# DigitalPhonetics/Intrinsic-Subgraph-Generation-for-VQA

Measured on AMD Instinct MI355X. Metric: GQA questions/sec, higher is better.
Workload: dtype f32

## Files before the change

intrinsic-subgraph-generation-for-vqa_amd/csrc/isg_layer_conv.hip:

```cpp
#include "isg_f16x3.hpp"

#include "isg_diag.hpp"
#include "isg_live_tables.hpp"
#include "../../include/isg_masked.h"

ISG_DIAG_BUFFER(g_lc_stamps)
#define LC_STAMP(i) ISG_DIAG_ADD(i)

namespace isg {

typedef __attribute__((address_space(3))) void lc_lds_t;
typedef __attribute__((address_space(1))) void lc_glb_t;

constexpr int LC_ROWS = 64, LC_ECAP = 256, LC_C = 128, LC_K = 128, LC_LDX = LC_C + 4, LC_LDA = LC_K + 8, LC_THREADS = 512;
constexpr int LC_OFF_XR = LC_ROWS * LC_LDX * 4;
constexpr int LC_OFF_A = 2 * LC_ROWS * LC_LDX * 4;
constexpr int LC_OFF_TAB = LC_OFF_A + 2 * 64 * LC_LDA * 2;
constexpr int LC_OFF_RAW = LC_OFF_TAB + 2 * (LC_ECAP * 16 + LC_ECAP * 4 + 68 * 4) + LC_ECAP * 4 + 4 * 64 * 4 + 64 * 4 + 3 * LC_C * 4 +
                           4 * LC_C * 4;
constexpr int LC_OFF_LIVE = LC_OFF_RAW + LC_ROWS * LC_K * 4;
constexpr int LC_SMEM_BYTES = LC_OFF_LIVE + 2 * 4 * 8;
static_assert(LC_OFF_RAW % 16 == 0, "16-byte pieces");
static_assert(LC_SMEM_BYTES <= 160 * 1024, "one workgroup per CU");

// ... 155 lines not shown
      const isg_f32x2 va = gelu_exact2(isg_f32x2{(acc[i][4 * g] * si) * wi4[g][0] + bv4[g][0], (acc[i][4 * g + 1] * si) * wi4[g][1] + bv4[g][1]});
      const isg_f32x2 vb = gelu_exact2(isg_f32x2{(acc[i][4 * g + 2] * si) * wi4[g][2] + bv4[g][2], (acc[i][4 * g + 3] * si) * wi4[g][3] + bv4[g][3]});
      *reinterpret_cast<hf32x4 *>(&sC[row][wave * 32 + 8 * g + 4 * hh]) = hf32x4{va.x, va.y, vb.x, vb.y};
    }
  }
  __syncthreads();
  const int grp = lane >> 4, l = lane & 15;
#pragma unroll
  for (int it = 0; it < 4; ++it) {
    const int n = wave * 16 + it * 4 + grp;
    float part = 0.f;
    if (n < nrows) {
      const float *qr = q + (int64_t)s_b[n] * NG_C;
      part += dot4_rn(*reinterpret_cast<const float4 *>(&sC[n][4 * l]), *reinterpret_cast<const float4 *>(qr + 4 * l));
      part += dot4_rn(*reinterpret_cast<const float4 *>(&sC[n][4 * (l + 16)]), *reinterpret_cast<const float4 *>(qr + 4 * (l + 16)));
    }
    const float dot = group_sum<16>(part);
    if (n < nrows && l == 0) gate[r0 + n] = gelu_libm(dot / denom);
  }
}

#define LC_EPILOGUE_ARITH(SL01, XS, XD)                                                                              \
    float part[4];                                                                                                   \
    int cb = tw * 32 + 4 * hh;        \
    asm volatile("" : "+v"(cb));                                                                                     \
    _Pragma("unroll") for (int g = 0; g < 4; ++g) {                                                                  \
      const int cc = cb + 8 * g;                                                                                     \
      const float4 xl4 = *reinterpret_cast<const float4 *>(&sXl[XS][cc]);                                            \
      const float4 xr4 = *reinterpret_cast<const float4 *>(&sXr[XD][cc]);                                            \
      const float4 at4 = *reinterpret_cast<const float4 *>(&s_att[cc]);                                              \
      const float4 wi4 = *reinterpret_cast<const float4 *>(&s_weinv[cc]);                                            \
      const float lv[4] = {xl4.x, xl4.y, xl4.z, xl4.w}, rv[4] = {xr4.x, xr4.y, xr4.z, xr4.w};                        \
      const float atv[4] = {at4.x, at4.y, at4.z, at4.w}, wiv[4] = {wi4.x, wi4.y, wi4.z, wi4.w};                      \
      part[g] = 0.f;                                                                                                 \
      _Pragma("unroll") for (int jj = 0; jj < 4; ++jj) {                                                             \
        const float e = (acc[g * 4 + jj] * sinv) * wiv[jj];                                                          \
        float z = (rv[jj] + lv[jj]) + e;                                                                             \
        if (MASKED) z *= me;                                                                                         \
        z = (SL01) ? fmaxf(z, z * slope) : (z > 0.f ? z : z * slope);    \
        if (MASKED) z *= me;                                                                                         \
        part[g] = fmaf(z, atv[jj], part[g]);                                                                         \
      }                                                                                                              \
      if (g < 3) __builtin_amdgcn_sched_barrier(0);                                                                  \
    }                                                                                                                \
    const float mine = (part[0] + part[1]) + (part[2] + part[3]);                                                    \
    const float tot = mine + __shfl_xor(mine, 32);                                                                   \
    if (hh == 0) s_part[tw * 64 + prow] = tot;

#define LC_AGGREGATE(REC)                                                                                                                  \
  {                                                                                                                                        \
    const int q8 = lane >> 3, j8 = lane & 7;                                                                                               \
    const int k = 8 * wave + q8;                                                                                                           \
    if (k < nrows) {                                                                                                                       \
      const int rb = s_rp[k], re = min(s_rp[k + 1], ne);                                                                                   \
      float lg4[4], e4[4];                                                                                                                 \
      int4 rc4[4];                                                                                                                         \
    _Pragma("unroll")                                                                                                                      \
      for (int u = 0; u < 4; ++u) {                                                                                                        \
        const int idx = max(min(rb + u, re - 1), 0);                                                                                       \
        lg4[u] = s_lg[idx];                                                                                                                \
        rc4[u] = REC(idx);                                                                                                                 \
      }                                                                                                                                    \
      float4 u2[2][4];                                                \
    _Pragma("unroll")                                                                                                                      \
      for (int u = 0; u < 2; ++u)                                                                                                          \
    _Pragma("unroll")                                                                                                                      \
        for (int m = 0; m < 4; ++m) u2[u][m] = *reinterpret_cast<const float4 *>(&sXl[rc4[u].x][32 * m + j8 * 4]);                         \
      float mx = fmaxf(fmaxf(-INFINITY, lg4[0]), fmaxf(fmaxf(lg4[1], lg4[2]), lg4[3]));                                                    \
    _Pragma("unroll 1")                                                                                                                    \
      for (int s = rb + 4; s < re; s += 4) {                                                                                               \
        const float v0 = s_lg[s], v1 = s_lg[min(s + 1, re - 1)], v2 = s_lg[min(s + 2, re - 1)], v3 = s_lg[min(s + 3, re - 1)];             \
        mx = fmaxf(fmaxf(mx, v0), fmaxf(fmaxf(v1, v2), v3));                                                                               \
      }                                                                                                                                    \
      float den = 0.f;                                             \
    _Pragma("unroll")                                                                                                                      \
      for (int u = 0; u < 4; ++u) {                                                                                                        \
        e4[u] = __builtin_amdgcn_exp2f((lg4[u] - mx) * 1.4426950408889634f);                                                               \
        den += rb + u < re ? e4[u] : 0.f;                                                                                                  \
      }                                                                                                                                    \
    _Pragma("unroll 1")                                                                                                                    \
      for (int s = rb + 4; s < re; s += 4) {                                                                                               \
        const float v0 = s_lg[s], v1 = s_lg[min(s + 1, re - 1)], v2 = s_lg[min(s + 2, re - 1)], v3 = s_lg[min(s + 3, re - 1)];             \
        const float e0 = __builtin_amdgcn_exp2f((v0 - mx) * 1.4426950408889634f);                                                          \
        const float e1 = __builtin_amdgcn_exp2f((v1 - mx) * 1.4426950408889634f);                                                          \
        const float e2 = __builtin_amdgcn_exp2f((v2 - mx) * 1.4426950408889634f);                                                          \
        const float e3 = __builtin_amdgcn_exp2f((v3 - mx) * 1.4426950408889634f);                                                          \
        den += e0;                                                                                                                         \
        den += s + 1 < re ? e1 : 0.f;                                                                                                      \
        den += s + 2 < re ? e2 : 0.f;                                                                                                      \
        den += s + 3 < re ? e3 : 0.f;                                                                                                      \
      }                                                                                                                                    \
      const float rden = __builtin_amdgcn_rcpf(den + 1e-16f);                                                                              \
      float4 o[4];                                                                                                                         \
    _Pragma("unroll")                                                                                                                      \
      for (int m = 0; m < 4; ++m) o[m] = make_float4(0.f, 0.f, 0.f, 0.f);                                                                  \
      int s = rb;                                                                                                                          \
    _Pragma("unroll 1")                                                                                                                    \
      while (true) {           \
        {                                           \
          const float wsel = (j8 & 2) ? ((j8 & 1) ? e4[3] : e4[2]) : ((j8 & 1) ? e4[1] : e4[0]);                                           \
          const int esel = (j8 & 2) ? ((j8 & 1) ? rc4[3].y : rc4[2].y) : ((j8 & 1) ? rc4[1].y : rc4[0].y);                                 \
          if (j8 < 4 && s + j8 < re) a.alpha[(int64_t)esel * a.H + hd] = wsel * rden;                                                      \
        }                                                                                                                                  \
    _Pragma("unroll")                                                                                                                      \
        for (int hp = 0; hp < 2; ++hp) {                                                                                                   \
          if (hp == 1) {                    \
// ... 11 lines not shown
            const float wm = MASKED ? mul_rn(w, __int_as_float(rc4[2 * hp + u].w)) : w;                                                    \
    _Pragma("unroll")                                                                                                                      \
            for (int m = 0; m < 4; ++m) {                                                                                                  \
              o[m].x = fmaf(u2[u][m].x, wm, o[m].x);                                                                                       \
              o[m].y = fmaf(u2[u][m].y, wm, o[m].y);                                                                                       \
              o[m].z = fmaf(u2[u][m].z, wm, o[m].z);                                                                                       \
              o[m].w = fmaf(u2[u][m].w, wm, o[m].w);                                                                                       \
            }                                                                                                                              \
          }                                                                                                                                \
        }                                                                                                                                  \
        s += 4;                                                                                                                            \
        if (s >= re) break;                                                                                                                \
    _Pragma("unroll")                                                                                                                      \
        for (int u = 0; u < 4; ++u) {                                                                                                      \
          const int idx = min(s + u, re - 1);                                                                                              \
          e4[u] = __builtin_amdgcn_exp2f((s_lg[idx] - mx) * 1.4426950408889634f);                                                          \
          rc4[u] = REC(idx);                                                                                                               \
        }                                                                                                                                  \
    _Pragma("unroll")                                                                                                                      \
        for (int u = 0; u < 2; ++u)                                                                                                        \
    _Pragma("unroll")                                                                                                                      \
          for (int m = 0; m < 4; ++m) u2[u][m] = *reinterpret_cast<const float4 *>(&sXl[rc4[u].x][32 * m + j8 * 4]);                       \
      }                                                                                                                                    \
      float rmx = 0.f;                                                                                                                     \
           \
            \
                                                                                   \
      unsigned zb = 0u;                                                                                                                    \
      if (MASKED) {                                                                                                                        \
    _Pragma("unroll")                                                                                                                      \
        for (int m = 0; m < 4; ++m)                                                                                                        \
          zb |= __float_as_uint(o[m].x) | __float_as_uint(o[m].y) | __float_as_uint(o[m].z) | __float_as_uint(o[m].w);                     \
      }                                                                                                                                    \
    _Pragma("unroll")                                                                                                                      \
      for (int m = 0; m < 4; ++m) {                                                                                                        \
        if (a.bias) {                                                                                                                      \
          const float4 b4 = *reinterpret_cast<const float4 *>(&s_bias[32 * m + j8 * 4]);                                                   \
          o[m].x += b4.x; o[m].y += b4.y; o[m].z += b4.z; o[m].w += b4.w;                                                                  \
        }                                                                                                                                  \
        hf32x4 o4 = {o[m].x, o[m].y, o[m].z, o[m].w};                                                                                      \
        __builtin_nontemporal_store(o4, reinterpret_cast<hf32x4 *>(a.out + (int64_t)(r0 + k) * a.ldo + hoff + 32 * m + j8 * 4));           \
        rmx = fmaxf(rmx, fmaxf(fmaxf(fabsf(o[m].x), fabsf(o[m].y)), fmaxf(fabsf(o[m].z), fabsf(o[m].w))));                                 \
      }                                                                                                                                    \
      if (a.rowmax) {                                                                                                                      \
        rmx = group_max<8>(rmx);                                                                                                           \
        if (j8 == 0) a.rowmax[(int64_t)(r0 + k) * a.H + hd] = rmx;                                                                         \
      }                                                                                                                                    \
      if (MASKED && a.row_dead) {                                                                                                          \
        zb |= (unsigned)dpp_mov_i<ISG_DPP_XOR1>((int)zb);                                                                                  \
        zb |= (unsigned)dpp_mov_i<ISG_DPP_XOR2>((int)zb);                                                                                  \
        zb |= (unsigned)dpp_mov_i<ISG_DPP_HMIRROR>((int)zb);                                                                               \
        if (j8 == 0) a.row_dead[(int64_t)(r0 + k) * a.H + hd] = zb == 0u ? 1 : 0;                                                          \
      }                                                                                                                                    \
    }                                                                                                                                      \
  }

template <bool MASKED, int KSE_T, bool SL01, bool LIVE>
__global__ __launch_bounds__(LC_THREADS, 2) void gatv2_layer_conv_kernel(LcArgs a) {
  extern __shared__ __attribute__((aligned(16))) unsigned char lc_smem[];
  typedef float (*BufX)[LC_LDX];
  typedef _Float16 (*BufP)[64][LC_LDA];
  BufX sXl = reinterpret_cast<BufX>(lc_smem);
  BufX sXr = reinterpret_cast<BufX>(lc_smem + LC_OFF_XR);
  BufP sA = reinterpret_cast<BufP>(lc_smem + LC_OFF_A);
  int4 *s_tab0 = reinterpret_cast<int4 *>(lc_smem + LC_OFF_TAB);
  float *s_einv0 = reinterpret_cast<float *>(s_tab0 + 2 * LC_ECAP);
  int *s_rp0 = reinterpret_cast<int *>(s_einv0 + 2 * LC_ECAP);
  float *s_lg = reinterpret_cast<float *>(s_rp0 + 2 * 68);
  float *s_part = s_lg + LC_ECAP;
  float *s_inv = s_part + 4 * 64;
  float *s_att = s_inv + 64, *s_weinv = s_att + LC_C;
  float *s_bias = s_weinv + LC_C, *s_bn = s_bias + LC_C, *s_wninv = s_bn + 2 * LC_C;
  unsigned long long *s_livew = reinterpret_cast<unsigned long long *>(lc_smem + LC_OFF_LIVE);
  constexpr bool cmp = MASKED && LIVE;

  const int bid = blockIdx.x;
  const int per_xcd = gridDim.x >> 3, jx = bid >> 3;
  const int hd = jx % a.H;
  const int ngrp = gridDim.x / a.H;
  int t = (bid & 7) * (per_xcd / a.H) + jx / a.H;
  const int T = *a.ntiles;
  if (t >= T) return;
  const int tid = threadIdx.x, lane = tid & 63;
  const int wave = __builtin_amdgcn_readfirstlane(tid >> 6);
  const int half = wave >> 2, tw = wave & 3;
  ISG_DIAG_BEGIN()
  const int fr = lane & 31, hh = lane >> 5, fk = hh * 8;
  const int hoff = hd * LC_C;
  const int srow = tid >> 5, scol = tid & 31, sc4 = scol;

  const int KSE = KSE_T ? KSE_T : a.KSE;
  const unsigned plane_e = (unsigned)a.NTE * (unsigned)KSE * 1024u;
  const __amdgpu_buffer_rsrc_t wrs_e =
      __builtin_amdgcn_make_buffer_rsrc(const_cast<_Float16 *>(a.We), 0, (int)(2u * plane_e), 0x00020000);
  const unsigned wb_e = (unsigned)(hd * (LC_C / 32) + tw) * (unsigned)KSE * 1024u;
  const int NTN = 2 * a.H * (LC_C / 32);
  const unsigned plane_n = (unsigned)NTN * 8u * 1024u;
  const __amdgpu_buffer_rsrc_t wrs_n =
      __builtin_amdgcn_make_buffer_rsrc(const_cast<_Float16 *>(a.Wn), 0, (int)(2u * plane_n), 0x00020000);
  const int ct = wave;
  const unsigned wb_n = (unsigned)((ct >> 2) * a.H * (LC_C / 32) + hd * (LC_C / 32) + (ct & 3)) * 8u * 1024u;
  hf16x8 wq_e[8][2], wq_n[8][2];
#pragma unroll
  for (int ks = 0; ks < 8; ++ks)
#pragma unroll
    for (int q = 0; q < 2; ++q) {
      wq_n[ks][q] = __builtin_bit_cast(hf16x8, __builtin_amdgcn_raw_buffer_load_b128(
                                                   wrs_n, lane * 16, (int)(wb_n + q * plane_n + (unsigned)ks * 1024u), 0));
// ... 235 lines not shown
      ISG_DIAG_KEEP2(acc[0], acc[15])
      LC_STAMP(3)
      if (MASKED && c + 1 == nchunk) LC_REQUEST_MASKS(desc_n)
      if (live) LC_EPILOGUE(c)
      __syncthreads();
      LC_STAMP(4)
      if (tid < 64 && 64 * c + tid < nact) {
        int slot = 64 * c + tid;
        if (cmp) { LC_LIVE() slot = lc_nth_live(lv, slot); }
        s_lg[slot] = (s_part[tid] + s_part[64 + tid]) + (s_part[128 + tid] + s_part[192 + tid]);
      }
    }
#undef LC_EPILOGUE
#undef LC_EPILOGUE_
#undef LC_LIVE
    LC_PLANES_LANDED()
    if (cmp && nchunk > 0) LC_BALLOT(desc_n, cur ^ 1)
    __syncthreads();

    LC_STAMP(11)
    if (nchunk == 0) {
      LC_REQUEST_TILE(desc_n)
      LC_REQUEST_MASKS(desc_n)
      LC_PLANES_LANDED()
      if (cmp) LC_BALLOT(desc_n, cur ^ 1)
      __syncthreads();
    }
    LC_STORE_TILE(desc_n, cur ^ 1)
    LC_REQUEST_PLANES(desc_n, cur ^ 1)
    LC_STAMP(5)
#define LC_REC_TAB(i) s_tab[i]
    LC_AGGREGATE(LC_REC_TAB)
#undef LC_REC_TAB
    LC_STAMP(6)
    if (!has_next) break;
    desc = desc_n;
    t = t_next;
    cur ^= 1;
  }
#undef LC_REQUEST_TILE
#undef LC_REQUEST_PLANES
#undef LC_REQUEST_MASKS
#undef LC_BALLOT
#undef LC_STORE_TILE
#undef LC_PLANES_LANDED
  ISG_DIAG_DUMP(g_lc_stamps, bid * 8 + wave, 12, )
}

constexpr int LG_MAXG = 6, LC_GROUP_DEFAULT = 6;
static_assert(LT_ROWS == LC_ROWS && LT_ECAP == LC_ECAP, "the table sets are cut for this kernel's tiles");
constexpr int LG_OFF_T = LC_OFF_A + 2 * 64 * LC_LDA * 2;
constexpr int LG_OFF_MISC = LG_OFF_T + LG_MAXG * LG_TILE_BYTES;
constexpr int LG_MISC_FLOATS = 4 * 64 + 3 * LC_C + 4 * LC_C + 64;
constexpr int LG_SMEM_BYTES = LG_OFF_MISC + LG_MISC_FLOATS * 4 + LG_MAXG * 16 + LG_MAXG * 8 + LG_MAXG * 4 * 8;
static_assert(LG_TILE_BYTES % 16 == 0 && LG_OFF_T % 16 == 0 && LG_OFF_MISC % 16 == 0 && LG_T_RP + 64 * 4 == 4 * 1024 &&
                  LG_TILE_BYTES == 4 * 1024 + 5 * 16 && LG_H_DESC == 4096 + 16 && LG_H_TOUCH == 4096 + 32 && LG_H_LIVE == 4096 + 48,
              "16-byte pieces; the fetch of a table set from memory: four 1 KiB pieces, then five 16-byte ones");
static_assert(64 * 512 <= 2 * 64 * LC_LDA * 2, "the node planes fit the panel image they share LDS with");
static_assert(LG_SMEM_BYTES <= 160 * 1024, "one workgroup per CU");

template <int KSE_T, bool SL01, bool TABLES>
__global__ __launch_bounds__(LC_THREADS, 2) void gatv2_layer_conv_groups_kernel(LcArgs a) {
  extern __shared__ __attribute__((aligned(16))) unsigned char lc_smem[];
  typedef float (*BufX)[LC_LDX];
  typedef _Float16 (*BufP)[64][LC_LDA];
  constexpr bool MASKED = true;
  BufX sXl = reinterpret_cast<BufX>(lc_smem);
  BufX sXr = reinterpret_cast<BufX>(lc_smem + LC_OFF_XR);
  BufP sA = reinterpret_cast<BufP>(lc_smem + LC_OFF_A);
  unsigned char *s_tiles = lc_smem + LG_OFF_T;
#define LG_EM(j) reinterpret_cast<int2 *>(s_tiles + (j) * LG_TILE_BYTES)
#define LG_LG(j) reinterpret_cast<float *>(s_tiles + (j) * LG_TILE_BYTES + LG_T_LG)
#define LG_SP(j) (s_tiles + (j) * LG_TILE_BYTES + LG_T_SP)
#define LG_DR(j) (s_tiles + (j) * LG_TILE_BYTES + LG_T_DR)
#define LG_LV(j) (s_tiles + (j) * LG_TILE_BYTES + LG_T_LV)
#define LG_RP(j) reinterpret_cast<int *>(s_tiles + (j) * LG_TILE_BYTES + LG_T_RP)
#define LG_POS(j) (s_tiles + (j) * LG_TILE_BYTES + LG_T_POS)
  float *s_part = reinterpret_cast<float *>(lc_smem + LG_OFF_MISC);
  float *s_att = s_part + 4 * 64, *s_weinv = s_att + LC_C;
  float *s_bias = s_weinv + LC_C, *s_bn = s_bias + LC_C, *s_wninv = s_bn + 2 * LC_C;
  int *s_nodes = reinterpret_cast<int *>(s_wninv + 2 * LC_C);
  int4 *s_desc = reinterpret_cast<int4 *>(s_nodes + 64);
  unsigned long long *s_touch = reinterpret_cast<unsigned long long *>(s_desc + LG_MAXG);
  unsigned long long *s_livew = s_touch + LG_MAXG;

  const int bid = blockIdx.x;
  const int per_xcd = gridDim.x >> 3, jx = bid >> 3;
  const int hd = jx % a.H;
  const int ngrp = gridDim.x / a.H;
  const int t = (bid & 7) * (per_xcd / a.H) + jx / a.H;
  const int T = *a.ntiles;
  if (t >= T) return;
  const int tid = threadIdx.x, lane = tid & 63;
  const int wave = __builtin_amdgcn_readfirstlane(tid >> 6);
  const int half = wave >> 2, tw = wave & 3;
  ISG_DIAG_BEGIN()
  const int fr = lane & 31, hh = lane >> 5, fk = hh * 8;
  const int hoff = hd * LC_C;
  const int srow = tid >> 5, sc4 = tid & 31;
  const int G = min(max(a.G, 1), LG_MAXG);

  const int KSE = KSE_T ? KSE_T : a.KSE;
  const unsigned plane_e = (unsigned)a.NTE * (unsigned)KSE * 1024u;
  const __amdgpu_buffer_rsrc_t wrs_e =
      __builtin_amdgcn_make_buffer_rsrc(const_cast<_Float16 *>(a.We), 0, (int)(2u * plane_e), 0x00020000);
  const unsigned wb_e = (unsigned)(hd * (LC_C / 32) + tw) * (unsigned)KSE * 1024u;
  const int NTN = 2 * a.H * (LC_C / 32);
  const unsigned plane_n = (unsigned)NTN * 8u * 1024u;
  const __amdgpu_buffer_rsrc_t wrs_n =
      __builtin_amdgcn_make_buffer_rsrc(const_cast<_Float16 *>(a.Wn), 0, (int)(2u * plane_n), 0x00020000);
  const int ct = wave;
  const unsigned wb_n = (unsigned)((ct >> 2) * a.H * (LC_C / 32) + hd * (LC_C / 32) + (ct & 3)) * 8u * 1024u;
  hf16x8 wq_e[8][2], wq_n[8][2];
#pragma unroll
  for (int ks = 0; ks < 8; ++ks)
#pragma unroll
    for (int q = 0; q < 2; ++q) {
      wq_n[ks][q] = __builtin_bit_cast(hf16x8, __builtin_amdgcn_raw_buffer_load_b128(
                                                   wrs_n, lane * 16, (int)(wb_n + q * plane_n + (unsigned)ks * 1024u), 0));
      wq_e[ks][q] = hf16x8{0, 0, 0, 0, 0, 0, 0, 0};
      if (ks < KSE)
        wq_e[ks][q] = __builtin_bit_cast(hf16x8, __builtin_amdgcn_raw_buffer_load_b128(
                                                     wrs_e, lane * 16, (int)(wb_e + q * plane_e + (unsigned)ks * 1024u), 0));
    }
  if (tid < LC_C) {
    s_att[tid] = a.att[hoff + tid];
    s_weinv[tid] = a.we_inv[hoff + tid];
    s_bias[tid] = a.bias ? a.bias[hoff + tid] : 0.f;
    sXl[0][tid] = 0.f;
  } else if (tid < 3 * LC_C) {
    const int c = tid - LC_C;
    const int src_col = (c >> 7) * a.H * LC_C + hoff + (c & 127);
    s_bn[c] = a.bn[src_col];
    s_wninv[c] = a.wn_inv[src_col];
  }
  const float slope = a.slope;
  const int prow = half * 32 + fr;

#pragma unroll 1
  for (int tg = t; tg < T; tg += G * ngrp) {
    int tl = tid, ll = lane;
    asm volatile("" : "+v"(tl), "+v"(ll));
    int ng = 0;
    if constexpr (TABLES) {
#pragma unroll
      for (int j = 0; j < LG_MAXG; ++j) ng += j < G && tg + j * ngrp < T ? 1 : 0;
      __syncthreads();
#pragma unroll 1
      for (int u = wave; u < 4 * ng; u += LC_THREADS / 64) {
        const int j = u >> 2, pc = u & 3;
        const unsigned char *img = a.live_tables + (size_t)(tg + j * ngrp) * LG_TILE_BYTES;
        __builtin_amdgcn_global_load_lds((lc_glb_t *)(img + pc * 1024 + ll * 16), (lc_lds_t *)(s_tiles + j * LG_TILE_BYTES + pc * 1024),
                                         16, 0, 0);
      }
      if (tl < 5 * ng) {
        const int j = tl / 5, pc = tl - 5 * j;
        const uint4 v = *reinterpret_cast<const uint4 *>(a.live_tables + (size_t)(tg + j * ngrp) * LG_TILE_BYTES + 4096 + pc * 16);
        const unsigned long long lo = (unsigned long long)v.x | ((unsigned long long)v.y << 32),
                                 hi = (unsigned long long)v.z | ((unsigned long long)v.w << 32);
        if (pc == 0) {
          *reinterpret_cast<uint4 *>(s_tiles + j * LG_TILE_BYTES + 4096) = v;
        } else if (pc == 1) {
          s_desc[j] = make_int4((int)v.x, (int)v.y, (int)v.z, (int)v.w);
        } else if (pc == 2) {
          s_touch[j] = lo;
        } else {
          s_livew[j * 4 + 2 * (pc - 3)] = lo;
          s_livew[j * 4 + 2 * (pc - 3) + 1] = hi;
        }
      }
      ISG_WAIT(0x0F70);
      __syncthreads();
    } else {
      int4 dsc[LG_MAXG];
#pragma unroll
      for (int j = 0; j < LG_MAXG; ++j) {
        const int tj = tg + j * ngrp;
        const bool on = j < G && tj < T;
        const int4 d = a.tile_info[min(tj, T - 1)];
        dsc[j] = make_int4(on ? __builtin_amdgcn_readfirstlane(d.x) : 0, on ? min(__builtin_amdgcn_readfirstlane(d.y), LC_ROWS) : 0,
                           on ? __builtin_amdgcn_readfirstlane(d.z) : 0, on ? min(__builtin_amdgcn_readfirstlane(d.w), LC_ECAP) : 0);
        ng += on ? 1 : 0;
      }
      int srcv[LG_MAXG], eidv[LG_MAXG], dstv[LG_MAXG], rpv[LG_MAXG];
      float einvv[LG_MAXG], mskv[LG_MAXG];
#pragma unroll
      for (int j = 0; j < LG_MAXG; ++j) {
        srcv[j] = eidv[j] = dstv[j] = rpv[j] = 0;
        einvv[j] = 1.f;
        if (j < ng) {
          if (tl <= dsc[j].y) rpv[j] = a.rowptr[dsc[j].x + tl];
          if (tl < dsc[j].w) {
            srcv[j] = a.src[dsc[j].z + tl];
            eidv[j] = a.eid[dsc[j].z + tl];
            dstv[j] = a.dst[dsc[j].z + tl];
            einvv[j] = a.ep_inv[dsc[j].z + tl];
          }
        }
      }
      if (tl < LG_MAXG) s_touch[tl] = 0ull;
      __syncthreads();
#pragma unroll
      for (int j = 0; j < LG_MAXG; ++j) {
        mskv[j] = 1.f;
        if (j < ng && tl < dsc[j].w)
          mskv[j] = a.edge_mask ? a.edge_mask[eidv[j]] : a.node_mask[srcv[j]] * a.node_mask[dstv[j]];
      }
#pragma unroll
      for (int j = 0; j < LG_MAXG; ++j) {
        if (j < ng) {
          const int r0n = dsc[j].x, nrn = dsc[j].y, e0n = dsc[j].z, nen = dsc[j].w;
          if (tl <= nrn) LG_RP(j)[tl] = rpv[j] - e0n;
          if (tl == 0) s_desc[j] = dsc[j];
          if (tl < LC_ECAP) {
            const int sx = min(max(srcv[j] - r0n, 0), max(nrn - 1, 0));
            const int dz = min(max(dstv[j] - r0n, 0), max(nrn - 1, 0));
            const bool lv = tl < nen && (__float_as_int(mskv[j]) & 0x7fffffff) != 0;
            const unsigned long long bw = __ballot(lv);
            if (ll == 0) s_livew[j * 4 + wave] = bw;
            if (lv) atomicOr(&s_touch[j], (1ull << sx) | (1ull << dz));
            LG_EM(j)[tl] = make_int2(eidv[j], __float_as_int(mskv[j]));
            LG_LG(j)[tl] = lv ? einvv[j] : 0.f;
            LG_SP(j)[tl] = (unsigned char)sx;
            LG_DR(j)[tl] = (unsigned char)dz;
          }
        }
      }
      __syncthreads();
    }
    LC_STAMP(0)

    int ntot = 0;
#pragma unroll
    for (int j = 0; j < LG_MAXG; ++j) ntot += j < ng ? __builtin_amdgcn_readfirstlane(__popcll(s_touch[j])) : 0;
    const int step = ntot <= LC_ROWS ? ng : 1;
#pragma unroll 1
    for (int ja = 0; ja < ng; ja += step) {
      const int jb = min(ja + step, ng);
      int cum[LG_MAXG];
      int nl = 0, nlive = 0;
#pragma unroll
      for (int j = 0; j < LG_MAXG; ++j) {
        if (j >= ja && j < jb) {
          const unsigned long long m = s_touch[j];
          if (tl < LC_ROWS) {
            const bool on = (m >> tl) & 1ull;
            const int p = nl + __popcll(m & ((1ull << tl) - 1ull));
            LG_POS(j)[tl] = (unsigned char)(on ? p : 0);
            if (on) s_nodes[p] = s_desc[j].x + tl;
          }
          int c[4];
#pragma unroll
          for (int i = 0; i < 4; ++i) {
            const unsigned long long w = s_livew[j * 4 + i];
            c[i] = __builtin_amdgcn_readfirstlane(__popc((unsigned)w) + __popc((unsigned)(w >> 32)));
          }
          if constexpr (!TABLES) {
            if (tl < LC_ECAP) {
              const unsigned long long w = s_livew[j * 4 + wave];
              const int pre = (wave > 0 ? c[0] : 0) + (wave > 1 ? c[1] : 0) + (wave > 2 ? c[2] : 0);
              if ((w >> ll) & 1ull) LG_LV(j)[pre + __popcll(w & ((1ull << ll) - 1ull))] = (unsigned char)tl;
            }
          }
          nl += __builtin_amdgcn_readfirstlane(__popcll(m));
          nlive += (c[0] + c[1]) + (c[2] + c[3]);
        }
        cum[j] = nlive;
      }
#define LG_FIND(k, jj, slot, e0v)                                                                                    \
  int jj = 0, slot, e0v;                                                                                             \
  {                                                                                                                  \
    int base_ = 0;                                                                                                   \
    _Pragma("unroll") for (int j_ = 0; j_ < LG_MAXG - 1; ++j_) {                                                     \
      const bool up_ = (k) >= cum[j_];                                                                               \
      jj += up_ ? 1 : 0;                                                                                             \
      base_ = up_ ? cum[j_] : base_;                                                                                 \
    }                                                                                                                \
    slot = LG_LV(jj)[(k) - base_];                                                                                   \
    e0v = s_desc[jj].z;                                                                                              \
  }
      __syncthreads();
      LC_STAMP(1)
#pragma unroll
      for (int j = 0; j < LG_MAXG; ++j)
        if (j >= ja && j < jb && tid < LC_ECAP) LG_SP(j)[tid] = LG_POS(j)[LG_SP(j)[tid]];
      if (nlive == 0) {
        __syncthreads();
      } else {
        const bool two = nl > 32;
#pragma unroll
        for (int u = 0; u < 4; ++u) {
          if (u < 2 || two) {
            const int lrow = srow + 16 * u;
            const int row = min(s_nodes[min(lrow, nl - 1)], a.N - 1);
            const int piece = (sc4 & 15) ^ (lrow & 15);
            __builtin_amdgcn_global_load_lds((lc_glb_t *)(a.xp + (int64_t)row * 256 + (sc4 >> 4) * 128 + piece * 8),
                                             (lc_lds_t *)(lc_smem + LC_OFF_A + (2 * wave + 16 * u) * 512), 16, 0, 0);
          }
        }
        float si2[2];
#pragma unroll
        for (int i = 0; i < 2; ++i) si2[i] = a.xinv[min(s_nodes[min(i * 32 + fr, nl - 1)], a.N - 1)];
        hf32x4 ra[4];
#pragma unroll
        for (int u = 0; u < 4; ++u) {
          LG_FIND(min(srow + 16 * u, nlive - 1), jj, slot, e0v)
          ra[u] = *reinterpret_cast<const hf32x4 *>(a.ep + (int64_t)(e0v + slot) * 256 + sc4 * 8);
        }
        ISG_WAIT(0x0F70);
        __syncthreads();
        LC_STAMP(2)
        {
          hf32x16 accn[2];
#pragma unroll
          for (int i = 0; i < 2; ++i)
#pragma unroll
            for (int r = 0; r < 16; ++r) accn[i][r] = 0.f;
#pragma unroll
          for (int i = 0; i < 2; ++i) {
            if (i == 0 || two) {
              hf16x8 an[2];
              hf32x16 c = accn[i];
#pragma unroll
              for (int ks = 0; ks < 8; ++ks) {
#pragma unroll
                for (int q = 0; q < 2; ++q)
                  an[q] = *reinterpret_cast<const hf16x8 *>(lc_smem + LC_OFF_A + (i * 32 + fr) * 512 + q * 256 + (((ks * 2 + hh) ^ (fr & 15)) << 4));
                c = __builtin_amdgcn_mfma_f32_32x32x16_f16(wq_n[ks][1], an[0], c, 0, 0, 0);
                c = __builtin_amdgcn_mfma_f32_32x32x16_f16(wq_n[ks][0], an[1], c, 0, 0, 0);
                c = __builtin_amdgcn_mfma_f32_32x32x16_f16(wq_n[ks][0], an[0], c, 0, 0, 0);
              }
              accn[i] = c;
            }
          }
          ISG_DIAG_KEEP2(accn[0][0], accn[1][15])
          LC_STAMP(8)
          __syncthreads();
          float(*dstx)[LC_LDX] = ct < 4 ? sXl : sXr;
// ... 29 lines not shown
            for (int u = 0; u < 4; ++u) *reinterpret_cast<hf32x4 *>(&sA[sc4 >> 4][srow + 16 * u][(sc4 & 15) * 8]) = ra[u];
            __syncthreads();
            LC_STAMP(10)
          }
          if (c + 1 < nchunk) {
#pragma unroll
            for (int u = 0; u < 4; ++u) {
              LG_FIND(min(64 * (c + 1) + srow + 16 * u, nlive - 1), jj, slot, e0v)
              ra[u] = *reinterpret_cast<const hf32x4 *>(a.ep + (int64_t)(e0v + slot) * 256 + sc4 * 8);
            }
          }
          const bool live = half == 0 || 64 * c + 32 < nlive;
          if (live) {
#pragma unroll
            for (int r = 0; r < 16; ++r) acc[r] = 0.f;
            hf16x8 af[2][2];
#pragma unroll
            for (int q = 0; q < 2; ++q) af[0][q] = *reinterpret_cast<const hf16x8 *>(&sA[q][prow][fk]);
#pragma unroll
            for (int ks = 0; ks < 8; ++ks) {
              if (ks < KSE) {
                if (ks + 1 < 8) {
#pragma unroll
                  for (int q = 0; q < 2; ++q)
                    af[(ks + 1) & 1][q] = *reinterpret_cast<const hf16x8 *>(&sA[q][prow][(ks + 1) * 16 + fk]);
                }
                acc = __builtin_amdgcn_mfma_f32_32x32x16_f16(wq_e[ks][0], af[ks & 1][1], acc, 0, 0, 0);
                acc = __builtin_amdgcn_mfma_f32_32x32x16_f16(wq_e[ks][1], af[ks & 1][0], acc, 0, 0, 0);
                acc = __builtin_amdgcn_mfma_f32_32x32x16_f16(wq_e[ks][0], af[ks & 1][0], acc, 0, 0, 0);
              }
            }
            ISG_DIAG_KEEP2(acc[0], acc[15])
            LC_STAMP(3)
            LG_FIND(min(64 * c + prow, nlive - 1), jj, slot, e0v)
            (void)e0v;
            const float sinv = LG_LG(jj)[slot];
            const int2 em = LG_EM(jj)[slot];
            const int xs = LG_SP(jj)[slot], xd = LG_POS(jj)[LG_DR(jj)[slot]];
            const float me = own_reg(__int_as_float(em.y));
            LC_EPILOGUE_ARITH(SL01, xs, xd)
          }
          __syncthreads();
          LC_STAMP(4)
          if (tid < 64 && 64 * c + tid < nlive) {
            LG_FIND(64 * c + tid, jj, slot, e0v)
            (void)e0v;
            LG_LG(jj)[slot] = (s_part[tid] + s_part[64 + tid]) + (s_part[128 + tid] + s_part[192 + tid]);
          }
        }
        __syncthreads();
        LC_STAMP(11)
      }
#undef LG_FIND
#pragma unroll 1
      for (int j = ja; j < jb; ++j) {
        const int4 dj = s_desc[j];
        const int r0 = __builtin_amdgcn_readfirstlane(dj.x), nrows = __builtin_amdgcn_readfirstlane(dj.y),
                  ne = __builtin_amdgcn_readfirstlane(dj.w);
        const float *s_lg = LG_LG(j);
        const int *s_rp = LG_RP(j);
        const int2 *s_em = LG_EM(j);
        const unsigned char *s_sp = LG_SP(j);
#define LG_REC(i) make_int4((int)s_sp[i], s_em[i].x, 0, s_em[i].y)
        LC_AGGREGATE(LG_REC)
#undef LG_REC
      }
      LC_STAMP(6)
    }
  }
#undef LG_EM
#undef LG_LG
#undef LG_SP
#undef LG_DR
#undef LG_LV
#undef LG_RP
#undef LG_POS
  ISG_DIAG_DUMP(g_lc_stamps, bid * 8 + wave, 12, )
}
#undef LC_AGGREGATE
#undef LC_EPILOGUE_ARITH

}

using namespace isg;

ISG_DIAG_SETTER(isg_lc_set_stamp_buffer, g_lc_stamps)

extern "C" int isg_instr_gate_planes(const float *x, const float *instr, const int64_t *batch, float *out, uint16_t *planes,
                                     float *inv_scale, int64_t N, int32_t C, void *stream) {
  if (N < 0 || C <= 0) return ISG_EINVAL;
  if (C != LC_K || (reinterpret_cast<uintptr_t>(x) & 15) != 0 || (reinterpret_cast<uintptr_t>(instr) & 15) != 0 ||
      (out && (reinterpret_cast<uintptr_t>(out) & 15) != 0) || (reinterpret_cast<uintptr_t>(planes) & 15) != 0 || N >= (1ll << 31))
    return ISG_EUNSUPPORTED;
  if (N == 0) return ISG_OK;
  if (!x || !instr || !batch || !planes || !inv_scale) return ISG_EINVAL;
  instr_gate_planes_kernel<<<(unsigned)((N + 7) / 8), 256, 0, as_stream(stream)>>>(x, instr, batch, out, reinterpret_cast<_Float16 *>(planes),
                                                                                   inv_scale, (int)N);
  return check_launch();
}

extern "C" int isg_node_gate_planes(const uint16_t *x_planes, const float *x_inv_scale, const uint16_t *w_frag, const float *w_inv_scale,
                                    const float *b, const float *q, const int64_t *batch, int32_t double_index, float *gate,
                                    int64_t N, int32_t C, void *stream) {
  if (N < 0 || C <= 0) return ISG_EINVAL;
  auto mis = [](const void *p) { return (reinterpret_cast<uintptr_t>(p) & 15) != 0; };
  if (C != NG_C || mis(x_planes) || mis(w_inv_scale) || mis(b) || mis(q) || N >= (1ll << 31)) return ISG_EUNSUPPORTED;
  if (N == 0) return ISG_OK;
  if (!x_planes || !x_inv_scale || !w_frag || !w_inv_scale || !b || !q || !batch || !gate) return ISG_EINVAL;
  node_gate_planes_kernel<<<(unsigned)((N + NG_ROWS - 1) / NG_ROWS), 256, 0, as_stream(stream)>>>(
      reinterpret_cast<const _Float16 *>(x_planes), x_inv_scale, reinterpret_cast<const _Float16 *>(w_frag), w_inv_scale, b, q,
      reinterpret_cast<const long long *>(batch), double_index, gate, (int)N, sqrtf((float)C));
  return check_launch();
}

static int lc_group_rule(int64_t N, int64_t E, int32_t H, int64_t max_tiles, int *gpx_out) {
  static const int force_group = [] { const char *e = getenv("ISG_LC_GROUP"); return e ? atoi(e) : 0; }();
  const int cus = device_cus();
  int gpx = (cus / 8) / H;
  if (gpx < 1) gpx = 1;
  const long long need = (max_tiles + 7) / 8;
  if (gpx > need) gpx = (int)need;
  if (gpx < 1) gpx = 1;
  if (gpx_out) *gpx_out = gpx;
  const long long tiles = std::max((N + LC_ROWS - 1) / LC_ROWS, (E + LC_ECAP - 1) / LC_ECAP);
  const long long per_wg = (std::min<long long>(tiles, max_tiles) + 8 * gpx - 1) / (8 * gpx);
  return force_group > 0 ? std::min(force_group, LG_MAXG) : (int)std::max<long long>(1, std::min<long long>(LC_GROUP_DEFAULT, per_wg));
}

static int lc_launch(const uint16_t *x_planes, const float *x_inv_scale, const uint16_t *wn_frag, const float *wn_inv_scale,
                     const float *bn, const uint16_t *edge_planes, const float *edge_inv_scale, const uint16_t *we_frag,
                     const float *we_inv_scale, const float *att, const float *bias, const int32_t *rowptr, const int32_t *eid,
                     const int32_t *src, const int32_t *dst, const int32_t *tile_info, const int32_t *ntiles, int64_t max_tiles,
                     const float *node_mask, const float *edge_mask, float *out, int32_t ldo, float *alpha, float *rowmax,
                     uint8_t *row_dead, const uint8_t *live_tables, int64_t N, int64_t E, int32_t H, int32_t C, int32_t K_in,
                     int32_t K_edge, float negative_slope, void *stream) {
  if (N < 0 || E < 0 || H <= 0 || C <= 0 || K_in <= 0 || K_edge <= 0 || max_tiles < 0 || ldo < H * C) return ISG_EINVAL;
  auto mis = [](const void *p) { return (reinterpret_cast<uintptr_t>(p) & 15) != 0; };
  if (C != LC_C || K_in != LC_K || K_edge > LC_K || (K_edge & 3) != 0 || (ldo & 3) != 0 || H > 16 || mis(x_planes) ||
      mis(edge_planes) || mis(out) || (bias && mis(bias)) || mis(tile_info) || mis(live_tables) || N >= (1ll << 31) ||
      E >= (1ll << 31))
    return ISG_EUNSUPPORTED;
  if (N == 0 || max_tiles == 0) return ISG_OK;
  if (!x_planes || !x_inv_scale || !wn_frag || !wn_inv_scale || !bn ||
      (E > 0 && (!edge_planes || !edge_inv_scale || !eid || !src || !dst || !alpha)) || !we_frag || !we_inv_scale || !att || !rowptr ||
      !tile_info || !ntiles || !out)
    return ISG_EINVAL;
  static const bool dense_mask = [] { const char *e = getenv("ISG_LC_DENSE_MASK"); return e && atoi(e) != 0; }();
  if (!isg_layer_conv_live_tables_enabled()) live_tables = nullptr;
  LcArgs a = {
      .xp = reinterpret_cast<const _Float16 *>(x_planes), .xinv = x_inv_scale, .Wn = reinterpret_cast<const _Float16 *>(wn_frag),
      .wn_inv = wn_inv_scale, .bn = bn, .ep = reinterpret_cast<const _Float16 *>(edge_planes), .ep_inv = edge_inv_scale,
      .We = reinterpret_cast<const _Float16 *>(we_frag), .we_inv = we_inv_scale, .att = att, .bias = bias, .rowptr = rowptr,
      .eid = eid, .src = src, .dst = dst, .ntiles = ntiles, .tile_info = reinterpret_cast<const int4 *>(tile_info),
      .edge_mask = edge_mask, .node_mask = node_mask, .out = out, .alpha = alpha, .rowmax = rowmax, .N = (int)N, .E = (int)E,
      .H = H, .KSE = (K_edge + 15) / 16, .NTE = H * C / 32, .ldo = ldo, .slope = negative_slope, .row_dead = row_dead, .G = 1,
      .live_tables = live_tables};
  if (!a.xp || !a.xinv || !a.Wn || !a.wn_inv || !a.bn || (a.E > 0 && (!a.ep || !a.ep_inv || !a.eid || !a.src || !a.dst || !a.alpha)) ||
      !a.We || !a.we_inv || !a.att || !a.rowptr || !a.tile_info || !a.ntiles || !a.out)
    return ISG_EINVAL;
  int gpx = 1;
  a.G = lc_group_rule(N, E, H, max_tiles, &gpx);
  const unsigned grid = 8u * (unsigned)H * (unsigned)gpx;
  hipStream_t st = as_stream(stream);
#define LC_LAUNCH_GT(KT, SL, TB)                                                                                     \
  {                                                                                                                  \
    if (!dyn_lds_ok<&gatv2_layer_conv_groups_kernel<KT, SL, TB>>(LG_SMEM_BYTES)) return ISG_EUNSUPPORTED;            \
    gatv2_layer_conv_groups_kernel<KT, SL, TB><<<grid, LC_THREADS, LG_SMEM_BYTES, st>>>(a);                          \
  }
#define LC_LAUNCH_G(KT, SL)                                                                                          \
  {                                                                                                                  \
    if (a.live_tables) LC_LAUNCH_GT(KT, SL, true) else LC_LAUNCH_GT(KT, SL, false)                                   \
  }
#define LC_LAUNCH(M, KT, SL, LV)                                                                                     \
  {                                                                                                                  \
    if (!dyn_lds_ok<&gatv2_layer_conv_kernel<M, KT, SL, LV>>(LC_SMEM_BYTES)) return ISG_EUNSUPPORTED;                \
    gatv2_layer_conv_kernel<M, KT, SL, LV><<<grid, LC_THREADS, LC_SMEM_BYTES, st>>>(a);                              \
  }
#define LC_LAUNCH_M(KT, SL)                                                                                          \
  {                                                                                                                  \
    if (dense_mask) LC_LAUNCH(true, KT, SL, false) else if (a.G > 1) LC_LAUNCH_G(KT, SL) else LC_LAUNCH(true, KT, SL, true) \
  }
  const bool masked = node_mask || edge_mask;
  const bool sl01 = negative_slope >= 0.f && negative_slope <= 1.f;
  if (a.KSE == 8 && sl01) {
    if (masked) LC_LAUNCH_M(8, true) else LC_LAUNCH(false, 8, true, false)
  } else if (sl01) {
    if (masked) LC_LAUNCH_M(0, true) else LC_LAUNCH(false, 0, true, false)
  } else {
    if (masked) LC_LAUNCH_M(0, false) else LC_LAUNCH(false, 0, false, false)
  }
#undef LC_LAUNCH_M
#undef LC_LAUNCH_G
#undef LC_LAUNCH_GT
#undef LC_LAUNCH
  return check_launch();
}

extern "C" int isg_gatv2_layer_conv(const uint16_t *x_planes, const float *x_inv_scale, const uint16_t *wn_frag, const float *wn_inv_scale,
                                    const float *bn, const uint16_t *edge_planes, const float *edge_inv_scale, const uint16_t *we_frag,
                                    const float *we_inv_scale, const float *att, const float *bias, const int32_t *rowptr,
                                    const int32_t *eid, const int32_t *src, const int32_t *dst, const int32_t *tile_info,
                                    const int32_t *ntiles, int64_t max_tiles, const float *node_mask, const float *edge_mask,
                                    float *out, int32_t ldo, float *alpha, float *rowmax, uint8_t *row_dead, int64_t N, int64_t E,
                                    int32_t H,
                                    int32_t C, int32_t K_in, int32_t K_edge, float negative_slope, void *stream) {
  return lc_launch(x_planes, x_inv_scale, wn_frag, wn_inv_scale, bn, edge_planes, edge_inv_scale, we_frag, we_inv_scale, att, bias,
                   rowptr, eid, src, dst, tile_info, ntiles, max_tiles, node_mask, edge_mask, out, ldo, alpha, rowmax, row_dead,
                   nullptr, N, E, H, C, K_in, K_edge, negative_slope, stream);
}

extern "C" int isg_gatv2_layer_conv_tables(const uint16_t *x_planes, const float *x_inv_scale, const uint16_t *wn_frag,
                                           const float *wn_inv_scale, const float *bn, const uint16_t *edge_planes,
                                           const float *edge_inv_scale, const uint16_t *we_frag, const float *we_inv_scale,
                                           const float *att, const float *bias, const int32_t *rowptr, const int32_t *eid,
                                           const int32_t *src, const int32_t *dst, const int32_t *tile_info, const int32_t *ntiles,
                                           int64_t max_tiles, const float *node_mask, const float *edge_mask, float *out, int32_t ldo,
                                           float *alpha, float *rowmax, uint8_t *row_dead, const uint8_t *live_tables, int64_t N,
                                           int64_t E, int32_t H, int32_t C, int32_t K_in, int32_t K_edge, float negative_slope,
                                           void *stream) {
  return lc_launch(x_planes, x_inv_scale, wn_frag, wn_inv_scale, bn, edge_planes, edge_inv_scale, we_frag, we_inv_scale, att, bias,
                   rowptr, eid, src, dst, tile_info, ntiles, max_tiles, node_mask, edge_mask, out, ldo, alpha, rowmax, row_dead,
                   live_tables, N, E, H, C, K_in, K_edge, negative_slope, stream);
}

extern "C" int32_t isg_gatv2_layer_conv_group(int64_t N, int64_t E, int32_t H, int64_t max_tiles) {
  if (N <= 0 || E < 0 || H <= 0 || H > 16 || max_tiles <= 0) return 1;
  return lc_group_rule(N, E, H, max_tiles, nullptr);
}

extern "C" int32_t isg_layer_conv_live_tables_enabled(void) {
  static const bool on = [] { const char *e = getenv("ISG_LC_TABLES"); return !e || atoi(e) != 0; }();
  return on ? 1 : 0;
}

namespace isg {

constexpr int RO_ROWS = 64, RO_C = 128, RO_LDA = RO_C + 8, RO_LDC = RO_C + 4, RO_GPC = 128;
constexpr int RO_SMEM_BYTES = 2 * (2 * RO_ROWS * RO_LDA * 2) + (6 * 64 + RO_GPC + 4) * 4;
static_assert(RO_ROWS * RO_LDC * 4 <= 2 * RO_ROWS * RO_LDA * 2, "xn aliases the first plane image");

struct RoArgs {
  const float *x;
  const _Float16 *w1f, *w2f;
  const float *w1_inv, *b1, *w2_inv, *b2;
  const float *y_bound;
  const float *q;
// ... 259 lines not shown
```

Baseline: 3.463 million.

## Aggregate only live destination rows in grouped GATv2 conv; fill dead rows directly

```diff
diff --git a/intrinsic-subgraph-generation-for-vqa_amd/csrc/isg_layer_conv.hip b/intrinsic-subgraph-generation-for-vqa_amd/csrc/isg_layer_conv.hip
--- a/intrinsic-subgraph-generation-for-vqa_amd/csrc/isg_layer_conv.hip
+++ b/intrinsic-subgraph-generation-for-vqa_amd/csrc/isg_layer_conv.hip
@@ -231,6 +231,11 @@
     const int q8 = lane >> 3, j8 = lane & 7;                                                                                               \
     const int k = 8 * wave + q8;                                                                                                           \
     if (k < nrows) {                                                                                                                       \
+      LC_AGGREGATE_ROW(REC)                                                                                                                \
+    }                                                                                                                                      \
+  }
+#define LC_AGGREGATE_ROW(REC)                                                                                                              \
+    {                                                                                                                                      \
       const int rb = s_rp[k], re = min(s_rp[k + 1], ne);                                                                                   \
       float lg4[4], e4[4];                                                                                                                 \
       int4 rc4[4];                                                                                                                         \
@@ -348,8 +353,7 @@
         zb |= (unsigned)dpp_mov_i<ISG_DPP_HMIRROR>((int)zb);                                                                               \
         if (j8 == 0) a.row_dead[(int64_t)(r0 + k) * a.H + hd] = zb == 0u ? 1 : 0;                                                          \
       }                                                                                                                                    \
-    }                                                                                                                                      \
-  }
+    }
 
 template <bool MASKED, int KSE_T, bool SL01, bool LIVE>
 __global__ __launch_bounds__(LC_THREADS, 2) void gatv2_layer_conv_kernel(LcArgs a) {
@@ -691,14 +695,14 @@
 constexpr int LG_OFF_T = LC_OFF_A + 2 * 64 * LC_LDA * 2;
 constexpr int LG_OFF_MISC = LG_OFF_T + LG_MAXG * LG_TILE_BYTES;
 constexpr int LG_MISC_FLOATS = 4 * 64 + 3 * LC_C + 4 * LC_C + 64;
-constexpr int LG_SMEM_BYTES = LG_OFF_MISC + LG_MISC_FLOATS * 4 + LG_MAXG * 16 + LG_MAXG * 8 + LG_MAXG * 4 * 8;
+constexpr int LG_SMEM_BYTES = LG_OFF_MISC + LG_MISC_FLOATS * 4 + LG_MAXG * 16 + LG_MAXG * 8 + LG_MAXG * 4 * 8 + 2 * LG_MAXG * 8 + 64 * 2 + 16;
 static_assert(LG_TILE_BYTES % 16 == 0 && LG_OFF_T % 16 == 0 && LG_OFF_MISC % 16 == 0 && LG_T_RP + 64 * 4 == 4 * 1024 &&
                   LG_TILE_BYTES == 4 * 1024 + 5 * 16 && LG_H_DESC == 4096 + 16 && LG_H_TOUCH == 4096 + 32 && LG_H_LIVE == 4096 + 48,
               "16-byte pieces; the fetch of a table set from memory: four 1 KiB pieces, then five 16-byte ones");
 static_assert(64 * 512 <= 2 * 64 * LC_LDA * 2, "the node planes fit the panel image they share LDS with");
 static_assert(LG_SMEM_BYTES <= 160 * 1024, "one workgroup per CU");
 
-template <int KSE_T, bool SL01, bool TABLES>
+template <int KSE_T, bool SL01, bool TABLES, bool AGG_ALL>
 __global__ __launch_bounds__(LC_THREADS, 2) void gatv2_layer_conv_groups_kernel(LcArgs a) {
   extern __shared__ __attribute__((aligned(16))) unsigned char lc_smem[];
   typedef float (*BufX)[LC_LDX];
@@ -722,6 +726,9 @@
   int4 *s_desc = reinterpret_cast<int4 *>(s_nodes + 64);
   unsigned long long *s_touch = reinterpret_cast<unsigned long long *>(s_desc + LG_MAXG);
   unsigned long long *s_livew = s_touch + LG_MAXG;
+  unsigned long long *s_ldst0 = s_livew + 4 * LG_MAXG;
+  unsigned short *s_alist = reinterpret_cast<unsigned short *>(s_ldst0 + 2 * LG_MAXG);
+  float *s_fillmax = reinterpret_cast<float *>(s_alist + 64);
 
   const int bid = blockIdx.x;
   const int per_xcd = gridDim.x >> 3, jx = bid >> 3;
@@ -775,11 +782,30 @@
   }
   const float slope = a.slope;
   const int prow = half * 32 + fr;
+  if constexpr (!AGG_ALL) {
+    float zero = 0.f, fill_max = 0.f;
+    asm volatile("" : "+v"(zero));
+    const int j8 = lane & 7;
+#pragma unroll
+    for (int m = 0; m < 4; ++m) {
+      float4 o = make_float4(zero, zero, zero, zero);
+      if (a.bias) {
+        const float4 b4 = *reinterpret_cast<const float4 *>(a.bias + hoff + 32 * m + j8 * 4);
+        o.x += b4.x; o.y += b4.y; o.z += b4.z; o.w += b4.w;
+      }
+      fill_max = fmaxf(fill_max, fmaxf(fmaxf(fabsf(o.x), fabsf(o.y)), fmaxf(fabsf(o.z), fabsf(o.w))));
+    }
+    fill_max = group_max<8>(fill_max);
+    if (tid == 0) *s_fillmax = fill_max;
+  }
+  int par = 0;
 
 #pragma unroll 1
   for (int tg = t; tg < T; tg += G * ngrp) {
     int tl = tid, ll = lane;
     asm volatile("" : "+v"(tl), "+v"(ll));
+    unsigned long long *s_ldst = s_ldst0 + par * LG_MAXG;
+    par ^= 1;
     int ng = 0;
     if constexpr (TABLES) {
 #pragma unroll
@@ -837,7 +863,16 @@
           }
         }
       }
-      if (tl < LG_MAXG) s_touch[tl] = 0ull;
+      if constexpr (AGG_ALL) {
+        if (tl < LG_MAXG) s_touch[tl] = 0ull;
+      } else {
+        unsigned zz = 0u;
+        asm volatile("" : "+v"(zz));
+        if (tl < LG_MAXG) {
+          s_touch[tl] = (unsigned long long)zz << 32 | zz;
+          s_ldst[tl] = (unsigned long long)zz << 32 | zz;
+        }
+      }
       __syncthreads();
 #pragma unroll
       for (int j = 0; j < LG_MAXG; ++j) {
@@ -858,6 +893,9 @@
             const unsigned long long bw = __ballot(lv);
             if (ll == 0) s_livew[j * 4 + wave] = bw;
             if (lv) atomicOr(&s_touch[j], (1ull << sx) | (1ull << dz));
+            if constexpr (!AGG_ALL) {
+              if (lv) atomicOr(&s_ldst[j], 1ull << dz);
+            }
             LG_EM(j)[tl] = make_int2(eidv[j], __float_as_int(mskv[j]));
             LG_LG(j)[tl] = lv ? einvv[j] : 0.f;
             LG_SP(j)[tl] = (unsigned char)sx;
@@ -901,6 +939,22 @@
               if ((w >> ll) & 1ull) LG_LV(j)[pre + __popcll(w & ((1ull << ll) - 1ull))] = (unsigned char)tl;
             }
           }
+          if constexpr (TABLES && !AGG_ALL) {
+            if (wave == j + 1) {
+              int rl = ll;
+              asm volatile("" : "+v"(rl));
+              const int4 dj = s_desc[j];
+              const int rb = rl < dj.y ? LG_RP(j)[rl] : 0, re = rl < dj.y ? min(LG_RP(j)[rl + 1], dj.w) : 0;
+              bool any = false;
+#pragma unroll
+              for (int i = 0; i < 4; ++i) {
+                const int lo = min(max(rb - 64 * i, 0), 64), hi = min(max(re - 64 * i, 0), 64);
+                if (hi > lo) any |= ((s_livew[j * 4 + i] >> lo) << (lo + 64 - hi)) != 0ull;
+              }
+              const unsigned long long rows = __ballot(any);
+              if (ll == 0) s_ldst[j] = rows;
+            }
+          }
           nl += __builtin_amdgcn_readfirstlane(__popcll(m));
           nlive += (c[0] + c[1]) + (c[2] + c[3]);
         }
@@ -923,6 +977,20 @@
 #pragma unroll
       for (int j = 0; j < LG_MAXG; ++j)
         if (j >= ja && j < jb && tid < LC_ECAP) LG_SP(j)[tid] = LG_POS(j)[LG_SP(j)[tid]];
+      int nagg = 0;
+      if constexpr (!AGG_ALL) {
+        unsigned long long lm[LG_MAXG];
+#pragma unroll
+        for (int j = 0; j < LG_MAXG; ++j) lm[j] = s_ldst[j];
+#pragma unroll
+        for (int j = 0; j < LG_MAXG; ++j) {
+          const unsigned long long m = j >= ja && j < jb ? lm[j] : 0ull;
+          const int p = nagg + __popcll(m & ((1ull << ll) - 1ull));
+          if (wave == j && ((m >> ll) & 1ull) && p < LC_ROWS) s_alist[p] = (unsigned short)(j << 8 | ll);
+          nagg += __builtin_amdgcn_readfirstlane(__popcll(m));
+        }
+        nagg = min(nagg, LC_ROWS);
+      }
       if (nlive == 0) {
         __syncthreads();
       } else {
@@ -1058,20 +1126,82 @@
         LC_STAMP(11)
       }
 #undef LG_FIND
+#define LG_REC(i) make_int4((int)s_sp[i], s_em[i].x, 0, s_em[i].y)
+      if constexpr (AGG_ALL) {
 #pragma unroll 1
-      for (int j = ja; j < jb; ++j) {
-        const int4 dj = s_desc[j];
-        const int r0 = __builtin_amdgcn_readfirstlane(dj.x), nrows = __builtin_amdgcn_readfirstlane(dj.y),
-                  ne = __builtin_amdgcn_readfirstlane(dj.w);
-        const float *s_lg = LG_LG(j);
-        const int *s_rp = LG_RP(j);
-        const int2 *s_em = LG_EM(j);
-        const unsigned char *s_sp = LG_SP(j);
-#define LG_REC(i) make_int4((int)s_sp[i], s_em[i].x, 0, s_em[i].y)
-        LC_AGGREGATE(LG_REC)
+        for (int j = ja; j < jb; ++j) {
+          const int4 dj = s_desc[j];
+          const int r0 = __builtin_amdgcn_readfirstlane(dj.x), nrows = __builtin_amdgcn_readfirstlane(dj.y),
+                    ne = __builtin_amdgcn_readfirstlane(dj.w);
+          const float *s_lg = LG_LG(j);
+          const int *s_rp = LG_RP(j);
+          const int2 *s_em = LG_EM(j);
+          const unsigned char *s_sp = LG_SP(j);
+          LC_AGGREGATE(LG_REC)
+        }
+        LC_STAMP(6)
+      } else {
+        int ft = tl;
+        asm volatile("" : "+v"(ft));
+        const int fc4 = ft & 31, frow = ft >> 5;
+        hf32x4 fill4 = {0.f, 0.f, 0.f, 0.f};
+        if (a.bias) {
+          float zero = 0.f;
+          asm volatile("" : "+v"(zero));
+          const float4 b4 = *reinterpret_cast<const float4 *>(&s_bias[fc4 * 4]);
+          fill4 = hf32x4{zero + b4.x, zero + b4.y, zero + b4.z, zero + b4.w};
+        }
+        const float fill_max = *s_fillmax;
+#pragma unroll 1
+        for (int j = ja; j < jb; ++j) {
+          const int4 dj = s_desc[j];
+          const int r0 = __builtin_amdgcn_readfirstlane(dj.x), nrows = __builtin_amdgcn_readfirstlane(dj.y),
+                    ne = __builtin_amdgcn_readfirstlane(dj.w);
+          const unsigned long long m = s_ldst[j];
+#pragma unroll
+          for (int u = 0; u < LC_ROWS * 32 / LC_THREADS; ++u) {
+            const int k = frow + u * (LC_THREADS / 32);
+            if (k < nrows && !((m >> k) & 1ull))
+              __builtin_nontemporal_store(fill4, reinterpret_cast<hf32x4 *>(a.out + (int64_t)(r0 + k) * a.ldo + hoff + fc4 * 4));
+          }
+          if (ft < LC_ECAP) {
+            if (ft < ne) {
+              const int dz = LG_DR(j)[ft];
+              if (!((m >> dz) & 1ull)) {
+                const int n = min(LG_RP(j)[dz + 1], ne) - LG_RP(j)[dz];
+                a.alpha[(int64_t)LG_EM(j)[ft].x * a.H + hd] = __builtin_amdgcn_rcpf((float)n + 1e-16f);
+              }
+            }
+          } else if (ft < LC_ECAP + LC_ROWS) {
+            const int k = ft - LC_ECAP;
+            if (k < nrows && !((m >> k) & 1ull)) {
+              if (a.rowmax) a.rowmax[(int64_t)(r0 + k) * a.H + hd] = fill_max;
+              if (a.row_dead) a.row_dead[(int64_t)(r0 + k) * a.H + hd] = 1;
+            }
+          }
+        }
+        LC_STAMP(5)
+        {
+          const int q8 = ll >> 3;
+          int j8 = ll & 7;
+          asm volatile("" : "+v"(j8));
+          const int i = 8 * q8 + wave;
+          if (i < nagg) {
+            const int ent = s_alist[i];
+            const int k = ent & 255;
+            const unsigned char *tb = s_tiles + (ent >> 8) * LG_TILE_BYTES;
+            const int4 dj = s_desc[ent >> 8];
+            const int r0 = dj.x, ne = dj.w;
+            const float *s_lg = reinterpret_cast<const float *>(tb + LG_T_LG);
+            const int *s_rp = reinterpret_cast<const int *>(tb + LG_T_RP);
+            const int2 *s_em = reinterpret_cast<const int2 *>(tb);
+            const unsigned char *s_sp = tb + LG_T_SP;
+            LC_AGGREGATE_ROW(LG_REC)
+          }
+        }
+        LC_STAMP(7)
+      }
 #undef LG_REC
-      }
-      LC_STAMP(6)
     }
   }
 #undef LG_EM
@@ -1153,6 +1283,7 @@
     return ISG_EINVAL;
   static const bool dense_mask = [] { const char *e = getenv("ISG_LC_DENSE_MASK"); return e && atoi(e) != 0; }();
   if (!isg_layer_conv_live_tables_enabled()) live_tables = nullptr;
+  static const bool agg_all_rows = [] { const char *e = getenv("ISG_LC_AGG_ALL_ROWS"); return e && atoi(e) != 0; }();
   LcArgs a = {
       .xp = reinterpret_cast<const _Float16 *>(x_planes), .xinv = x_inv_scale, .Wn = reinterpret_cast<const _Float16 *>(wn_frag),
       .wn_inv = wn_inv_scale, .bn = bn, .ep = reinterpret_cast<const _Float16 *>(edge_planes), .ep_inv = edge_inv_scale,
@@ -1168,10 +1299,14 @@
   a.G = lc_group_rule(N, E, H, max_tiles, &gpx);
   const unsigned grid = 8u * (unsigned)H * (unsigned)gpx;
   hipStream_t st = as_stream(stream);
+#define LC_LAUNCH_GTA(KT, SL, TB, AA)                                                                                \
+  {                                                                                                                  \
+    if (!dyn_lds_ok<&gatv2_layer_conv_groups_kernel<KT, SL, TB, AA>>(LG_SMEM_BYTES)) return ISG_EUNSUPPORTED;        \
+    gatv2_layer_conv_groups_kernel<KT, SL, TB, AA><<<grid, LC_THREADS, LG_SMEM_BYTES, st>>>(a);                      \
+  }
 #define LC_LAUNCH_GT(KT, SL, TB)                                                                                     \
   {                                                                                                                  \
-    if (!dyn_lds_ok<&gatv2_layer_conv_groups_kernel<KT, SL, TB>>(LG_SMEM_BYTES)) return ISG_EUNSUPPORTED;            \
-    gatv2_layer_conv_groups_kernel<KT, SL, TB><<<grid, LC_THREADS, LG_SMEM_BYTES, st>>>(a);                          \
+    if (agg_all_rows) LC_LAUNCH_GTA(KT, SL, TB, true) else LC_LAUNCH_GTA(KT, SL, TB, false)                          \
   }
 #define LC_LAUNCH_G(KT, SL)                                                                                          \
   {                                                                                                                  \
@@ -1198,6 +1333,7 @@
 #undef LC_LAUNCH_M
 #undef LC_LAUNCH_G
 #undef LC_LAUNCH_GT
+#undef LC_LAUNCH_GTA
 #undef LC_LAUNCH
   return check_launch();
 }
```

Result: faster. 3.501 million (median of 6 runs) (+1.1%).
